# seceq/zkir

Hardware: AMD Instinct MI355X
Metric: trace rows/sec (2^20-cycle fib: execution-trace fill + BabyBear NTT/LDE + Poseidon2 Merkle commitment) (higher is better)
Workload: dtype u32 (Baby Bear, 31-bit modular) / u64 trace words

## Files before the change

### zkir_amd/build.py

```python
from __future__ import annotations

import os
import subprocess
import sys

HERE = os.path.dirname(os.path.abspath(__file__))
CSRC = os.path.join(HERE, "csrc")
OUT = os.path.join(HERE, "libzkir_amd.so")
OBJ = os.path.join(HERE, "build")

HOST_SOURCES = ["interp.cpp", "hashes.cpp", "verify.cpp"]
HIP_SOURCES = ["trace_fill.hip", "witness.hip", "ntt.hip", "stark.hip", "memcheck.hip", "abi.hip"]
HEADERS = ["host.h", "hashcall.h", "babybear.h", "poseidon2.h", "air.h", "stark_prove.inl", os.path.join("..", "..", "include", "zkir_amd.h"), os.path.join("..", "..", "include", "zkir_amd_experimental.h")]

HIPCC = os.environ.get("HIPCC", "/opt/rocm/bin/hipcc")
ARCH = "gfx950"
COMMON = ["-O3", "-std=c++17", "-fPIC", "-Wall", "-Wno-unused-function"]
EXTRA = {"stark.hip": ["-mllvm", "-amdgpu-sched-strategy=max-ilp"]}


def sources_sha16() -> str:
    import hashlib
    h = hashlib.sha256()
    for name in sorted(HIP_SOURCES + [x for x in HEADERS if not x.startswith("..")]):
# ... 22 lines not shown
        else:
            cmd = [HIPCC, "-x", "c++", *COMMON, "-march=x86-64-v2", *defines, "-c", src, "-o", obj]
        subprocess.check_call(cmd)
    out = os.path.join(HERE, "variants", f"libzkir_amd_{tag}.so")
    subprocess.check_call([HIPCC, f"--offload-arch={ARCH}", "-shared", "-fPIC", "-o", out, *objs])
    return out


PROBE_SRC = os.path.join(HERE, "..", "tests", "hip", "arith_probe.hip")
PROBE_OUT = os.path.join(HERE, "..", "tests", "hip", "libzkir_arith_probe.so")


def build_probe(force: bool = False, verbose: bool = False) -> str:
    src, out = os.path.normpath(PROBE_SRC), os.path.normpath(PROBE_OUT)
    deps = [os.path.join(CSRC, "babybear.h"), os.path.join(CSRC, "poseidon2.h")]
    if force or _newer(src, out, deps):
        cmd = [HIPCC, f"--offload-arch={ARCH}", *COMMON, *EXTRA["stark.hip"], "-shared", src, "-o", out]
        if verbose:
            print(" ".join(cmd), flush=True)
        subprocess.check_call(cmd)
    return out


def build(force: bool = False, verbose: bool = False) -> str:
    os.makedirs(OBJ, exist_ok=True)
    deps = [os.path.normpath(os.path.join(CSRC, h)) for h in HEADERS]
    objs, cmds = [], []
    for name in HOST_SOURCES + HIP_SOURCES:
        src = os.path.join(CSRC, name)
        obj = os.path.join(OBJ, name + ".o")
        objs.append(obj)
        if force or _newer(src, obj, deps):
            if name.endswith(".hip"):
                cmds.append([HIPCC, f"--offload-arch={ARCH}", *COMMON, *EXTRA.get(name, []), "-c", src, "-o", obj])
            else:
                cmds.append([HIPCC, "-x", "c++", *COMMON, "-march=x86-64-v2", "-c", src, "-o", obj])
    if cmds:
        from concurrent.futures import ThreadPoolExecutor
        def run(cmd):
            if verbose:
                print(" ".join(cmd), flush=True)
            subprocess.check_call(cmd)
        with ThreadPoolExecutor(max_workers=int(os.environ.get("ZKIR_BUILD_JOBS", "4"))) as ex:
            list(ex.map(run, cmds))
    if force or any(_newer(o, OUT, []) for o in objs):
        cmd = [HIPCC, f"--offload-arch={ARCH}", "-shared", "-fPIC", "-o", OUT, *objs]
        if verbose:
            print(" ".join(cmd), flush=True)
        subprocess.check_call(cmd)
    build_probe(force, verbose)
    return OUT


if __name__ == "__main__":
    print(build(force="--force" in sys.argv, verbose=True))
```

### zkir_amd/csrc/babybear.h

```cpp
#pragma once
#include <cstdint>

#if defined(__HIPCC__)
#define BB_HD __host__ __device__ __forceinline__
#else
#define BB_HD inline
#endif

namespace bb {

constexpr uint32_t P = 0x78000001u;
constexpr uint32_t NEG_PINV = 0x77FFFFFFu;
constexpr uint32_t R1 = 0x0FFFFFFEu;
constexpr uint32_t R2 = 0x45DDDDE3u;
constexpr uint32_t GEN = 31u;
constexpr uint32_t ROOT27 = 0x1A427A41u;
constexpr uint32_t W_EXT = 11u;

BB_HD uint32_t add(uint32_t a, uint32_t b) { const uint32_t s = a + b, d = s - P; return d < s ? d : s; }
BB_HD uint32_t sub(uint32_t a, uint32_t b) { const uint32_t d = a - b, e = d + P; return e < d ? e : d; }
BB_HD uint32_t neg(uint32_t a) { return a ? P - a : 0u; }
BB_HD uint32_t dbl(uint32_t a) { return add(a, a); }
BB_HD uint32_t mont_mul(uint32_t a, uint32_t b) {
  const uint64_t t = (uint64_t)a * b;
// ... 75 lines not shown
  return (uint32_t)((acc + (uint64_t)m * P) >> 32);
}
BB_HD int32_t smont_mul(int32_t a, int32_t b) {
  const int64_t t = (int64_t)a * b;
  const int32_t m = (int32_t)((uint32_t)t * NEG_PINV);
  return (int32_t)(((uint64_t)t + (uint64_t)((int64_t)m * (int64_t)P)) >> 32);
}
BB_HD int32_t smont_mul_add(int32_t a, int32_t b, uint64_t c) {
  const uint64_t t = (uint64_t)((int64_t)a * b) + c;
  const int32_t m = (int32_t)((uint32_t)t * NEG_PINV);
  return (int32_t)((t + (uint64_t)((int64_t)m * (int64_t)P)) >> 32);
}
BB_HD int32_t smont_reduce_wide(int64_t acc) {
  const int32_t m = (int32_t)((uint32_t)acc * NEG_PINV);
  return (int32_t)(((uint64_t)acc + (uint64_t)((int64_t)m * (int64_t)P)) >> 32);
}
BB_HD int64_t sacc_add(int64_t acc, int32_t x) {
#if defined(__HIP_DEVICE_COMPILE__)
  int64_t r;
  asm("v_mad_i64_i32 %0, vcc, %1, 1, %2" : "=v"(r) : "v"(x), "v"(acc) : "vcc");
  return r;
#else
  return acc + x;
#endif
}
BB_HD uint32_t to_mont(uint32_t a) { return mont_mul(a, R2); }
BB_HD uint32_t from_mont(uint32_t a) { return mont_mul(a, 1u); }
BB_HD uint32_t mul(uint32_t a, uint32_t b) { return mont_mul(mont_mul(a, b), R2); }
BB_HD uint32_t pow(uint32_t a, uint64_t e) {
  uint32_t r = R1, b = to_mont(a);
  while (e) { if (e & 1) r = mont_mul(r, b); b = mont_mul(b, b); e >>= 1; }
  return from_mont(r);
}
BB_HD uint32_t inv(uint32_t a) { return pow(a, P - 2); }
BB_HD uint32_t root_of_unity(int log_n) { uint32_t w = ROOT27; for (int i = log_n; i < 27; i++) w = mul(w, w); return w; }

struct E4 { uint32_t c[4]; };
BB_HD E4 e_add(const E4& a, const E4& b) { return E4{{add(a.c[0], b.c[0]), add(a.c[1], b.c[1]), add(a.c[2], b.c[2]), add(a.c[3], b.c[3])}}; }
BB_HD E4 e_sub(const E4& a, const E4& b) { return E4{{sub(a.c[0], b.c[0]), sub(a.c[1], b.c[1]), sub(a.c[2], b.c[2]), sub(a.c[3], b.c[3])}}; }
BB_HD E4 e_mul_m(const E4& a, const E4& b) {
  constexpr uint32_t W11M = (uint32_t)((11ull * R1) % P);
  const uint32_t a0 = a.c[0], a1 = a.c[1], a2 = a.c[2], a3 = a.c[3], b0 = b.c[0], b1 = b.c[1], b2 = b.c[2], b3 = b.c[3];
  const uint32_t t4 = add(add(mont_mul(a1, b3), mont_mul(a2, b2)), mont_mul(a3, b1));
  const uint32_t t5 = add(mont_mul(a2, b3), mont_mul(a3, b2));
  const uint32_t t6 = mont_mul(a3, b3);
  E4 r;
// ... 28 lines not shown
```

### zkir_amd/csrc/ntt.hip

```cpp
#include <hip/hip_runtime.h>

#include <atomic>
#include <cstdlib>
#include <mutex>
#include <type_traits>

#include "../../include/zkir_amd.h"
#include "../../include/zkir_amd_experimental.h"
#include "babybear.h"
#include "host.h"

namespace {

constexpr int NT = 256;
__device__ __forceinline__ uint32_t bitrev(uint32_t x, int bits) { return bits == 0 ? 0u : __brev(x) >> (32 - bits); }

template <int K, int N, class F>
__device__ __forceinline__ void static_for(F&& f) {
  if constexpr (K < N) { f(std::integral_constant<int, K>{}); static_for<K + 1, N>(f); }
}

using u32x4 = uint32_t __attribute__((ext_vector_type(4)));
__device__ __forceinline__ u32x4 ld4(const uint4* p) { return *reinterpret_cast<const u32x4*>(p); }
__device__ __forceinline__ void st4(uint4* p, u32x4 v) { *reinterpret_cast<u32x4*>(p) = v; }

__device__ __forceinline__ void wave_sync_lds() { asm volatile("s_waitcnt lgkmcnt(0)" ::: "memory"); }

__device__ __forceinline__ uint4 add4(uint4 a, uint4 b) { return make_uint4(bb::add(a.x, b.x), bb::add(a.y, b.y), bb::add(a.z, b.z), bb::add(a.w, b.w)); }
__device__ __forceinline__ uint4 sub4(uint4 a, uint4 b) { return make_uint4(bb::sub(a.x, b.x), bb::sub(a.y, b.y), bb::sub(a.z, b.z), bb::sub(a.w, b.w)); }
__device__ __forceinline__ uint4 addl4(uint4 a, uint4 b) { return make_uint4(a.x + b.x, a.y + b.y, a.z + b.z, a.w + b.w); }
__device__ __forceinline__ uint4 subl4(uint4 a, uint4 b) { return make_uint4(a.x - b.x + bb::P, a.y - b.y + bb::P, a.z - b.z + bb::P, a.w - b.w + bb::P); }
__device__ __forceinline__ uint4 mul4(uint4 a, uint32_t w) { return make_uint4(bb::mont_mul(a.x, w), bb::mont_mul(a.y, w), bb::mont_mul(a.z, w), bb::mont_mul(a.w, w)); }

__device__ __forceinline__ void dif4(uint4& x0, uint4& x1, uint4& x2, uint4& x3, uint32_t wA, uint32_t wB, uint32_t w2) {
  const uint4 y0 = add4(x0, x2), y2 = mul4(subl4(x0, x2), wA);
  const uint4 y1 = add4(x1, x3), y3 = mul4(subl4(x1, x3), wB);
  x0 = add4(y0, y1); x1 = mul4(subl4(y0, y1), w2);
  x2 = add4(y2, y3); x3 = mul4(subl4(y2, y3), w2);
}
__device__ __forceinline__ void dit4(uint4& x0, uint4& x1, uint4& x2, uint4& x3, uint32_t w1, uint32_t w2, uint32_t w2i) {
  const uint4 t1 = mul4(x1, w1), t3 = mul4(x3, w1);
  const uint4 y0 = add4(x0, t1), y1 = sub4(x0, t1), y2 = addl4(x2, t3), y3 = subl4(x2, t3);
  const uint4 u2 = mul4(y2, w2), u3 = mul4(y3, w2i);
  x0 = add4(y0, u2); x2 = sub4(y0, u2); x1 = add4(y1, u3); x3 = sub4(y1, u3);
}

template <bool DIT>
__global__ __launch_bounds__(NT) void ntt_stage_kernel(uint4* __restrict__ data, uint64_t blk_u4, int L, int s0, const uint32_t* __restrict__ tw) {
  uint4* x = data + (uint64_t)blockIdx.y * blk_u4;
  const uint64_t item = (uint64_t)blockIdx.x * NT + threadIdx.x;
  const uint32_t n = 1u << L;
  if (item >= (uint64_t)n) return;
  const uint32_t t = (uint32_t)(item >> 1), h = (uint32_t)(item & 1);
  uint32_t p, stride, w;
  if (DIT) { stride = 1u << s0; const uint32_t hi = t >> s0, lo = t & (stride - 1); p = (hi << (s0 + 1)) + lo; w = tw[lo << (L - s0 - 1)]; }
  else { stride = n >> (s0 + 1); const uint32_t hi = t / stride, lo = t % stride; p = hi * (n >> s0) + lo; w = tw[lo << s0]; }
  const uint4 a = x[(uint64_t)p * 2 + h], b = x[(uint64_t)(p + stride) * 2 + h];
  if (DIT) { const uint4 tt = mul4(b, w); x[(uint64_t)p * 2 + h] = add4(a, tt); x[(uint64_t)(p + stride) * 2 + h] = sub4(a, tt); }
  else { x[(uint64_t)p * 2 + h] = add4(a, b); x[(uint64_t)(p + stride) * 2 + h] = mul4(subl4(a, b), w); }
}

struct TraceSrc01 { zkir_trace_columns t; uint64_t n_real; };
__device__ __forceinline__ u32x4 trace_quad01(const TraceSrc01& q, uint32_t blk, uint32_t half, uint64_t i) {
  const bool pad = i >= q.n_real;
  const uint64_t src = pad ? q.n_real - 1 : i;
  u32x4 r;
  if (blk == 0 && half == 0) {
    const uint64_t pcv = q.t.pc[src];
    r.x = (uint32_t)((q.t.cycle[src] + (i - src)) % bb::P); r.y = (uint32_t)(pcv & 0xFFFFF); r.z = (uint32_t)((pcv >> 20) & 0xFFFFF); r.w = (uint32_t)(pcv >> 40);
  } else if (blk == 0) {
    const uint32_t w = q.t.instruction[src];
    r.x = w & 0x7F; r.y = (w >> 7) & 0xF; r.z = (w >> 11) & 0xF; r.w = (w >> 15) & 0xF;
  } else {
    auto limbs = [&](int g, uint32_t out[3]) {
      const uint64_t o = (uint64_t)g * q.t.reg_stride + src;
      const uint64_t v = q.t.registers[o];
      const int bits = q.t.reg_state[o] ? 30 : 20;
      const uint64_t mask = (1ull << bits) - 1;
      out[0] = (uint32_t)(v & mask); out[1] = (uint32_t)((v >> bits) & mask); out[2] = (uint32_t)(v >> (2 * bits));
    };
    uint32_t a[3], b[3];
    if (half == 0) { limbs(1, a); r.x = q.t.instruction[src] >> 19; r.y = a[0]; r.z = a[1]; r.w = a[2]; }
    else { limbs(2, a); limbs(3, b); r.x = a[0]; r.y = a[1]; r.z = a[2]; r.w = b[0]; }
  }
  return r;
}

template <bool DIT, int R, int C, int NTH, bool FUSED = false>
__global__ __launch_bounds__(NTH) void ntt_strided_r4_kernel(uint4* __restrict__ data, uint64_t blk_u4, uint32_t tiles_per_block, uint32_t total, int L, int s0,
                                                              const uint32_t* __restrict__ tw, const uint32_t* __restrict__ small, int log_small, uint32_t j4_m, TraceSrc01 fsrc = TraceSrc01{}) {
  constexpr int B = 2 * R;
  constexpr uint32_t POS = 1u << (B + C), QUADS = POS / 4, CMASK = (1u << C) - 1, PLANE = POS + 4;
  constexpr uint32_t MOVES = 2 * POS / NTH;
  static_assert(QUADS % NTH == 0 && NTH % (1 << C) == 0 && (2 * POS) % NTH == 0, "tile / thread geometry");
  extern __shared__ uint4 lds4[];
  const uint32_t n = 1u << L;
  const uint32_t stride_mid = DIT ? (1u << s0) : (n >> (s0 + B));
  const uint32_t lo_tiles = stride_mid >> C;
  auto geometry = [&](uint32_t w, uint4*& x, uint32_t& base, uint32_t& lo0) {
    const uint32_t tile = w % tiles_per_block;
    x = data + (uint64_t)(w / tiles_per_block) * blk_u4;
    const uint32_t hi = tile / lo_tiles;
    lo0 = (tile % lo_tiles) << C;
    base = (DIT ? (hi << (s0 + B)) : hi * (n >> s0)) + lo0;
  };
  static_assert(QUADS == NTH, "one quad per lane and round");
  u32x4 pre[MOVES];
  uint4* x; uint32_t base, lo0;
  uint32_t w = blockIdx.x;
  if (w >= total) return;
  uint32_t sm[R];
#pragma unroll
  for (int r = 0; r < R; r++) {
    const int b = 2 * r;
    const uint32_t qq = threadIdx.x >> C;
    if (!DIT) { const int lg = B - 2 - b; sm[r] = small[(qq & ((1u << lg) - 1)) << (log_small - (B - b))]; }
    else sm[r] = small[(qq & ((1u << b) - 1)) << (log_small - (b + 2))];
// ... 37 lines not shown
    }
#pragma unroll
    for (int r = 0; r < R; r++) {
      const int b = 2 * r;
#pragma unroll
      for (uint32_t k = 0; k < QUADS / NTH; k++) {
        const uint32_t q = threadIdx.x + k * NTH;
        const uint32_t lo_l = q & CMASK, qq = q >> C;
        uint32_t i0, d, wa, wb, wc;
        if (!DIT) {
          const int lg = B - 2 - b;
          const uint32_t h2 = 1u << lg, mid_lo = qq & (h2 - 1), mid_hi = qq >> lg;
          i0 = ((((mid_hi << (lg + 2)) | mid_lo)) << C) | lo_l; d = h2 << C;
          wa = bb::mont_mul(tp[r], sm[r]);
          wb = bb::mont_mul(wa, j4_m); wc = bb::mont_mul(wa, wa);
        } else {
          const uint32_t dm = 1u << b, mid_lo = qq & (dm - 1), mid_hi = qq >> b;
          i0 = ((((mid_hi << (b + 2)) | mid_lo)) << C) | lo_l; d = dm << C;
          wb = bb::mont_mul(tp[r], sm[r]);
          wa = bb::mont_mul(wb, wb); wc = bb::mont_mul(wb, j4_m);
        }
        uint4* pl0 = lds4; uint4* pl1 = lds4 + PLANE;
        uint4 x0 = pl0[i0], x1 = pl0[i0 + d], x2 = pl0[i0 + 2 * d], x3 = pl0[i0 + 3 * d];
        uint4 y0 = pl1[i0], y1 = pl1[i0 + d], y2 = pl1[i0 + 2 * d], y3 = pl1[i0 + 3 * d];
        if (!DIT) dif4(x0, x1, x2, x3, wa, wb, wc); else dit4(x0, x1, x2, x3, wa, wb, wc);
        pl0[i0] = x0; pl0[i0 + d] = x1; pl0[i0 + 2 * d] = x2; pl0[i0 + 3 * d] = x3;
        if (!DIT) dif4(y0, y1, y2, y3, wa, wb, wc); else dit4(y0, y1, y2, y3, wa, wb, wc);
        pl1[i0] = y0; pl1[i0 + d] = y1; pl1[i0 + 2 * d] = y2; pl1[i0 + 3 * d] = y3;
      }
      const bool wave_local = !DIT ? (r + 1 < R && B - 2 - b <= 6 - C) : (r + 1 < R && b + 2 <= 6 - C);
      if (wave_local) wave_sync_lds(); else __syncthreads();
    }
#pragma unroll
    for (uint32_t k = 0; k < MOVES; k++) {
      const uint32_t e = threadIdx.x + k * NTH, row = e >> (C + 1), wv = e & ((2u << C) - 1);
      x[((uint64_t)base + (uint64_t)row * stride_mid) * 2 + wv] = lds4[(wv & 1) * PLANE + ((row << C) | (wv >> 1))];
    }
    if (wn >= total) break;
    w = wn; x = xn; base = base_n; lo0 = lo0_n;
  }
}

template <bool DIT, int S>
__global__ __launch_bounds__(NT) void ntt_reg_kernel(uint4* __restrict__ data, uint64_t blk_u4, int L, int s0, const uint32_t* __restrict__ tw, uint32_t r4_m, uint32_t r8_m,
                                                       uint32_t r8_3_m) {
  constexpr int E = 1 << S;
  const uint32_t n = 1u << L;
  uint4* x = data + (uint64_t)blockIdx.y * blk_u4;
  const uint64_t item = (uint64_t)blockIdx.x * NT + threadIdx.x;
  if (item >= ((uint64_t)n >> S) * 2) return;
  const uint32_t t = (uint32_t)(item >> 1), h = (uint32_t)(item & 1);
  const uint32_t d = DIT ? (1u << s0) : (n >> (s0 + S));
  const uint32_t hi = t / d, lo = t % d;
  const uint64_t base = ((uint64_t)hi * d * E + lo) * 2 + h;
// ... 42 lines not shown
    } else {
      const uint32_t f1 = bb::mont_mul(Uf, r4_m);
#pragma unroll
      for (int g = 0; g < 4; g += 2) { const uint4 tt = mul4(v[g + 1], Um); const uint4 a = v[g]; v[g] = add4(a, tt); v[g + 1] = sub4(a, tt); }
      { const uint4 tt = mul4(v[2], Uf); const uint4 a = v[0]; v[0] = add4(a, tt); v[2] = sub4(a, tt); }
      { const uint4 tt = mul4(v[3], f1); const uint4 a = v[1]; v[1] = add4(a, tt); v[3] = sub4(a, tt); }
    }
  }
#pragma unroll
  for (int k = 0; k < E; k++) x[base + (uint64_t)k * d * 2] = v[k];
}

inline unsigned cu_count() {
  static std::mutex mu;
  static unsigned cached[64] = {};
  int dev = 0;
  if (hipGetDevice(&dev) != hipSuccess || dev < 0 || dev >= 64) return 256u;
  std::lock_guard<std::mutex> lk(mu);
  if (!cached[dev]) { hipDeviceProp_t p; cached[dev] = hipGetDeviceProperties(&p, dev) == hipSuccess && p.multiProcessorCount > 0 ? (unsigned)p.multiProcessorCount : 256u; }
  return cached[dev];
}
inline int persist() { static const int v = getenv("ZKIR_NTT_PERSIST") ? atoi(getenv("ZKIR_NTT_PERSIST")) : 1; return v; }

template <bool DIT, int R, int C, int NTH, bool FUSED = false>
void launch_strided_r4(uint32_t* data, uint64_t n, uint32_t n_blocks, int L, int s0, const uint32_t* tw, const uint32_t* small, int log_small, uint32_t j4_m, hipStream_t s,
                       const TraceSrc01* fsrc = nullptr) {
  constexpr size_t lds = 16u * 2 * ((1u << (2 * R + C)) + 4);
  auto k = ntt_strided_r4_kernel<DIT, R, C, NTH, FUSED>;
  static std::atomic<uint64_t> attr_done{0};
  int dev = 0; (void)hipGetDevice(&dev);
  const uint64_t bit = 1ull << (dev & 63);
  if (!(attr_done.load(std::memory_order_relaxed) & bit)) { (void)hipFuncSetAttribute(reinterpret_cast<const void*>(k), hipFuncAttributeMaxDynamicSharedMemorySize, (int)lds); attr_done.fetch_or(bit); }
  const uint32_t tiles = (uint32_t)(n >> (2 * R + C)), total = tiles * n_blocks;
  const unsigned per_cu = (unsigned)((160u << 10) / lds) > 0 ? (unsigned)((160u << 10) / lds) : 1u;
  unsigned grid = persist() ? cu_count() * (per_cu > 8 ? 8 : per_cu) : total;
  if (grid > total) grid = total;
  hipLaunchKernelGGL(k, dim3(grid), dim3(NTH), lds, s, (uint4*)data, 2 * n, tiles, total, L, s0, tw, small, log_small, j4_m, fsrc ? *fsrc : TraceSrc01{});
}

inline int strided_c() { static const int c = getenv("ZKIR_NTT_C") ? atoi(getenv("ZKIR_NTT_C")) : 2; return c; }

template <bool DIT>
void run_strided_stages(uint32_t* data, uint64_t n, uint32_t n_blocks, int L, int s0, int stages, const uint32_t* tw, const uint32_t* small, int log_small, uint32_t j4_m,
                        uint32_t r8_m, uint32_t r8_3_m, hipStream_t s) {
  while (stages > 0) {
    int take;
    if (stages >= 10 && stages != 11) take = 10;
    else if (stages == 11) take = 8;
    else if (stages == 9) take = 6;
    else if (stages == 7) take = 4;
    else if (stages == 5) take = 3;
    else take = stages;
    switch (take) {
      case 10:
        if (strided_c() == 2) launch_strided_r4<DIT, 5, 2, 1024>(data, n, n_blocks, L, s0, tw, small, log_small, j4_m, s);
        else launch_strided_r4<DIT, 5, 1, 512>(data, n, n_blocks, L, s0, tw, small, log_small, j4_m, s);
        break;
      case 8: launch_strided_r4<DIT, 4, 3, 512>(data, n, n_blocks, L, s0, tw, small, log_small, j4_m, s); break;
      case 6: launch_strided_r4<DIT, 3, 4, 256>(data, n, n_blocks, L, s0, tw, small, log_small, j4_m, s); break;
      case 4: launch_strided_r4<DIT, 2, 5, 128>(data, n, n_blocks, L, s0, tw, small, log_small, j4_m, s); break;
      case 3:
        hipLaunchKernelGGL((ntt_reg_kernel<DIT, 3>), dim3((unsigned)(((n >> 3) * 2 + NT - 1) / NT), n_blocks), dim3(NT), 0, s, (uint4*)data, 2 * n, L, s0, tw, j4_m, r8_m, r8_3_m);
        break;
      case 2:
        hipLaunchKernelGGL((ntt_reg_kernel<DIT, 2>), dim3((unsigned)(((n >> 2) * 2 + NT - 1) / NT), n_blocks), dim3(NT), 0, s, (uint4*)data, 2 * n, L, s0, tw, j4_m, r8_m, r8_3_m);
        break;
      default:
        hipLaunchKernelGGL(ntt_stage_kernel<DIT>, dim3((unsigned)((n + NT - 1) / NT), n_blocks), dim3(NT), 0, s, (uint4*)data, 2 * n, L, s0, tw);
        break;
    }
    s0 += take; stages -= take;
  }
}

__global__ __launch_bounds__(NT) void lde_small_kernel(const uint32_t* __restrict__ in, uint32_t* __restrict__ out, int L, const uint32_t* __restrict__ small_inv,
                                                        const uint32_t* __restrict__ small_fwd, const uint32_t* __restrict__ g_lo, const uint32_t* __restrict__ g_hi) {
  extern __shared__ uint32_t lds[];
  const uint32_t n = 1u << L;
  const uint32_t* x = in + (uint64_t)blockIdx.x * n * 8;
  uint32_t* y = out + (uint64_t)blockIdx.x * 2 * n * 8;
  for (int c = 0; c < 8; c++) {
    for (uint32_t e = threadIdx.x; e < n; e += NT) lds[e] = x[(uint64_t)e * 8 + c];
    __syncthreads();
// ... 11 lines not shown
    uint32_t v[2];
    int cnt = 0;
    for (uint32_t e = threadIdx.x; e < n; e += NT) { const uint32_t k = bitrev(e, L); v[cnt++] = bb::mont_mul(bb::mont_mul(lds[e], g_lo[k & 1023]), g_hi[k >> 10]); }
    __syncthreads();
    cnt = 0;
    for (uint32_t e = threadIdx.x; e < n; e += NT) { lds[2 * e] = v[cnt]; lds[2 * e + 1] = v[cnt]; cnt++; }
    __syncthreads();
    for (int s = 1; s <= L; s++) {
      const uint32_t half = 1u << s;
      for (uint32_t q = threadIdx.x; q < n; q += NT) {
        const uint32_t r_lo = q & (half - 1), r_hi = q >> s;
        const uint32_t ia = (r_hi << (s + 1)) | r_lo, ib = ia + half;
        const uint32_t a = lds[ia], t = bb::mont_mul(lds[ib], small_fwd[r_lo << (L - s)]);
        lds[ia] = bb::add(a, t); lds[ib] = bb::sub(a, t);
      }
      __syncthreads();
    }
    for (uint32_t e = threadIdx.x; e < 2 * n; e += NT) y[(uint64_t)e * 8 + c] = lds[e];
    __syncthreads();
  }
}

constexpr int MID_NT = 512;
__global__ __launch_bounds__(MID_NT) void lde_middle_r4_kernel(const uint4* __restrict__ in, uint4* __restrict__ out, uint32_t chunks_per_block, uint32_t total, int L,
                                                                const uint32_t* __restrict__ small_inv, const uint32_t* __restrict__ small_fwd,
                                                                const uint32_t* __restrict__ g_lo, const uint32_t* __restrict__ g_hi, uint32_t j4_inv_m, uint32_t j4_fwd_m) {
  constexpr int Bm = 10;
  constexpr uint32_t APL = 1024;
  __shared__ uint4 A[2 * APL];
  __shared__ uint4 Bf[2048];
  const uint32_t n = 1u << L, t = threadIdx.x;
  uint32_t w = blockIdx.x;
  if (w >= total) return;
  uint32_t tw_i[5], tw_f[5];
#pragma unroll
  for (int r = 0; r < 5; r++) {
    const int lg = 8 - 2 * r;
    tw_i[r] = small_inv[((t & 255) & ((1u << lg) - 1)) << (2 * r)];
    const int sft = 2 * r + 1;
    tw_f[r] = small_fwd[(t & ((1u << sft) - 1)) << (Bm - sft - 1)];
  }
  u32x4 pre[4];
  uint32_t glo[4], ghi[4];
  auto fetch = [&](uint32_t ww) {
    const uint4* x = in + ((uint64_t)(ww / chunks_per_block) * n + ((uint64_t)(ww % chunks_per_block) << Bm)) * 2;
#pragma unroll
    for (int k = 0; k < 4; k++) pre[k] = ld4(&x[t + k * MID_NT]);
// ... 21 lines not shown
        const int lg = 8 - 2 * r;
        const uint32_t h2 = 1u << lg, lo = q & (h2 - 1), hi = q >> lg;
        const uint32_t i0 = (hi << (lg + 2)) | lo;
        const uint32_t wA = tw_i[r];
        const uint32_t wB = bb::mont_mul(wA, j4_inv_m), w2 = bb::mont_mul(wA, wA);
        uint4 x0 = a[i0], x1 = a[i0 + h2], x2 = a[i0 + 2 * h2], x3 = a[i0 + 3 * h2];
        dif4(x0, x1, x2, x3, wA, wB, w2);
        if (r == 4) {
          x0 = mul4(x0, gs[0]); x1 = mul4(x1, gs[1]); x2 = mul4(x2, gs[2]); x3 = mul4(x3, gs[3]);
        }
        a[i0] = x0; a[i0 + h2] = x1; a[i0 + 2 * h2] = x2; a[i0 + 3 * h2] = x3;
        if (r >= 1 && r < 4) wave_sync_lds(); else __syncthreads();
      }
    }
#pragma unroll 1
    for (int h = 0; h < 2; h++) {
      const uint4* a = A + h * APL;
      uint4* F = h == 0 ? Bf : A;
#pragma unroll
      for (int r = 0; r < 5; r++) {
        const int s = 2 * r + 1;
        const uint32_t lo = t & ((1u << s) - 1), hi = t >> s;
        const uint32_t i0 = (hi << (s + 2)) | lo, d = 1u << s;
        const uint32_t w2 = tw_f[r];
        const uint32_t w1 = bb::mont_mul(w2, w2), w2i = bb::mont_mul(w2, j4_fwd_m);
        uint4 x0, x1, x2, x3;
        if (r == 0) {
          x0 = a[i0 >> 1]; x1 = a[(i0 + d) >> 1]; x2 = a[(i0 + 2 * d) >> 1]; x3 = a[(i0 + 3 * d) >> 1];
          __syncthreads();
        } else { x0 = F[i0]; x1 = F[i0 + d]; x2 = F[i0 + 2 * d]; x3 = F[i0 + 3 * d]; }
        dit4(x0, x1, x2, x3, w1, w2, w2i);
        F[i0] = x0; F[i0 + d] = x1; F[i0 + 2 * d] = x2; F[i0 + 3 * d] = x3;
        if (r < 2) wave_sync_lds(); else __syncthreads();
      }
    }
#pragma unroll
    for (int k = 0; k < 4; k++) { const uint32_t e = t + k * MID_NT; y[((uint64_t)2 * base + e) * 2] = Bf[e]; y[((uint64_t)2 * base + e) * 2 + 1] = A[e]; }
    __syncthreads();
    if (wn >= total) break;
    w = wn;
  }
}

}

namespace zkir {

void lde_run(const LdeTables& t, uint32_t* in, uint32_t n_blocks, uint32_t* out, void* stream) {
  hipStream_t s = (hipStream_t)stream;
  const int L = t.log_n;
  const uint32_t N = 1u << L;
  static const uint32_t j4_inv_m = bb::to_mont(bb::inv(bb::root_of_unity(2))), j4_fwd_m = bb::to_mont(bb::root_of_unity(2));
  static const uint32_t r8_fwd = bb::root_of_unity(3), r8_inv = bb::inv(r8_fwd);
  static const uint32_t r8_inv_m = bb::to_mont(r8_inv), r8_inv3_m = bb::to_mont(bb::mul(bb::mul(r8_inv, r8_inv), r8_inv));
  static const uint32_t r8_fwd_m = bb::to_mont(r8_fwd), r8_fwd3_m = bb::to_mont(bb::mul(bb::mul(r8_fwd, r8_fwd), r8_fwd));
  if (L < 10) {
    hipLaunchKernelGGL(lde_small_kernel, dim3(n_blocks), dim3(NT), (8u << L), s, in, out, L, t.small_inv, t.small_fwd, t.g_lo, t.g_hi);
    return;
  }
  run_strided_stages<false>(in, N, n_blocks, L, 0, L - 10, t.tw_inv, t.small_inv, 10, j4_inv_m, r8_inv_m, r8_inv3_m, s);
  {
    const uint32_t chunks = N >> 10, total = chunks * n_blocks;
    unsigned grid = persist() ? cu_count() * 2 : total;
    if (grid > total) grid = total;
    hipLaunchKernelGGL(lde_middle_r4_kernel, dim3(grid), dim3(MID_NT), 0, s, (const uint4*)in, (uint4*)out, chunks, total, L, t.small_inv, t.small_fwd, t.g_lo, t.g_hi,
                       j4_inv_m, j4_fwd_m);
  }
  run_strided_stages<true>(out, (uint64_t)2 * N, n_blocks, L + 1, 11, L - 10, t.tw_fwd, t.small_fwd, 11, j4_fwd_m, r8_fwd_m, r8_fwd3_m, s);
}


bool strided_variant_run(const LdeTables& t, uint32_t* data, uint32_t n_blocks, int variant, bool dit, void* stream) {
  hipStream_t s = (hipStream_t)stream;
  const int L = dit ? t.log_n + 1 : t.log_n;
  if (t.log_n < 20) return false;
  const uint64_t n = (uint64_t)1 << L;
  static const uint32_t j4_inv_m = bb::to_mont(bb::inv(bb::root_of_unity(2))), j4_fwd_m = bb::to_mont(bb::root_of_unity(2));
  const uint32_t* tw = dit ? t.tw_fwd : t.tw_inv; const uint32_t* sm = dit ? t.small_fwd : t.small_inv;
  const int ls = dit ? 11 : 10; const uint32_t j4 = dit ? j4_fwd_m : j4_inv_m; const int s0 = dit ? 11 : 0;
#define ZKIR_VARIANT(R, C, NTH) do { if (dit) launch_strided_r4<true, R, C, NTH>(data, n, n_blocks, L, s0, tw, sm, ls, j4, s); else launch_strided_r4<false, R, C, NTH>(data, n, n_blocks, L, s0, tw, sm, ls, j4, s); } while (0)
  switch (variant) {
    case 0: ZKIR_VARIANT(5, 2, 1024); break;
    case 1: ZKIR_VARIANT(5, 1, 512); break;
    case 2: ZKIR_VARIANT(4, 3, 512); break;
    case 3: ZKIR_VARIANT(4, 2, 256); break;
    case 4: ZKIR_VARIANT(3, 4, 256); break;
    default: return false;
  }
#undef ZKIR_VARIANT
  return true;
}

bool lde_run_fused01(const LdeTables& t, const zkir_trace_columns* trace, uint64_t n_real, uint32_t* in, uint32_t n_blocks, uint32_t* out, void* stream) {
  hipStream_t s = (hipStream_t)stream;
  const int L = t.log_n;
  if (L < 20 || L == 21 || n_blocks < 3 || strided_c() != 2) return false;
  const uint32_t N = 1u << L;
  static const uint32_t j4_inv_m = bb::to_mont(bb::inv(bb::root_of_unity(2))), j4_fwd_m = bb::to_mont(bb::root_of_unity(2));
  static const uint32_t r8_fwd = bb::root_of_unity(3), r8_inv = bb::inv(r8_fwd);
  static const uint32_t r8_inv_m = bb::to_mont(r8_inv), r8_inv3_m = bb::to_mont(bb::mul(bb::mul(r8_inv, r8_inv), r8_inv));
  static const uint32_t r8_fwd_m = bb::to_mont(r8_fwd), r8_fwd3_m = bb::to_mont(bb::mul(bb::mul(r8_fwd, r8_fwd), r8_fwd));
  const TraceSrc01 src{*trace, n_real};
  launch_strided_r4<false, 5, 2, 1024, true>(in, N, 2, L, 0, t.tw_inv, t.small_inv, 10, j4_inv_m, s, &src);
  launch_strided_r4<false, 5, 2, 1024>(in + (uint64_t)2 * N * 8, N, n_blocks - 2, L, 0, t.tw_inv, t.small_inv, 10, j4_inv_m, s);
  if (L - 10 > 10) run_strided_stages<false>(in, N, n_blocks, L, 10, L - 20, t.tw_inv, t.small_inv, 10, j4_inv_m, r8_inv_m, r8_inv3_m, s);
  {
    const uint32_t chunks = N >> 10, total = chunks * n_blocks;
    unsigned grid = persist() ? cu_count() * 2 : total;
    if (grid > total) grid = total;
    hipLaunchKernelGGL(lde_middle_r4_kernel, dim3(grid), dim3(MID_NT), 0, s, (const uint4*)in, (uint4*)out, chunks, total, L, t.small_inv, t.small_fwd, t.g_lo, t.g_hi,
                       j4_inv_m, j4_fwd_m);
  }
  run_strided_stages<true>(out, (uint64_t)2 * N, n_blocks, L + 1, 11, L - 10, t.tw_fwd, t.small_fwd, 11, j4_fwd_m, r8_fwd_m, r8_fwd3_m, s);
  return true;
}

}
```

Before: 185.6 million.

## Use signed wide-accumulator radix-4 DIT butterflies with deferred canonicalisation in forward NTT

Replaces the forward (DIT) radix-4 butterfly in the strided and LDE-middle kernels with a signed 64-bit accumulation scheme. Twiddles are centred to signed values and products are accumulated with v_mad_i64_i32, and reductions happen only twice per butterfly instead of after every add/sub. Outputs stay in a signed redundant range and are canonicalised only on the final round of the last forward pass. Results go to LDS through hand-written ds_write2 stores. The aim is fewer modular add/sub/reduce instructions, at the cost of complex bound reasoning, more inline asm, and sched barriers that may limit compiler scheduling. It also adds an NTT probe build target.

```diff
diff --git a/zkir_amd/build.py b/zkir_amd/build.py
--- a/zkir_amd/build.py
+++ b/zkir_amd/build.py
@@ -68,6 +68,20 @@
     return out
 
 
+NTT_PROBE_SRC = os.path.join(HERE, "..", "tests", "hip", "ntt_probe.hip")
+NTT_PROBE_OUT = os.path.join(HERE, "..", "tests", "hip", "libzkir_ntt_probe.so")
+
+
+def build_ntt_probe(force: bool = False, verbose: bool = False) -> str:
+    src, out = os.path.normpath(NTT_PROBE_SRC), os.path.normpath(NTT_PROBE_OUT)
+    if force or _newer(src, out, [os.path.join(CSRC, "babybear.h")]):
+        cmd = [HIPCC, f"--offload-arch={ARCH}", *COMMON, *EXTRA.get("ntt.hip", []), "-shared", src, "-o", out]
+        if verbose:
+            print(" ".join(cmd), flush=True)
+        subprocess.check_call(cmd)
+    return out
+
+
 def build(force: bool = False, verbose: bool = False) -> str:
     os.makedirs(OBJ, exist_ok=True)
     deps = [os.path.normpath(os.path.join(CSRC, h)) for h in HEADERS]
@@ -95,6 +109,7 @@
             print(" ".join(cmd), flush=True)
         subprocess.check_call(cmd)
     build_probe(force, verbose)
+    build_ntt_probe(force, verbose)
     return OUT
 
 
diff --git a/zkir_amd/csrc/babybear.h b/zkir_amd/csrc/babybear.h
--- a/zkir_amd/csrc/babybear.h
+++ b/zkir_amd/csrc/babybear.h
@@ -121,6 +121,76 @@
   return r;
 #else
   return acc + x;
+#endif
+}
+namespace wq {
+constexpr int64_t W_MAX = (P - 1) / 2;
+constexpr int64_t X_ANY = (int64_t)1 << 31;
+constexpr int64_t RED_DOMAIN = (int64_t)(((uint64_t)1 << 63) - ((uint64_t)P << 31));
+constexpr int64_t red_bound(int64_t acc) { return (acc + ((int64_t)P << 31)) >> 32; }
+constexpr int64_t layer1_acc_bound(int64_t x) { return x * ((int64_t)R1 + W_MAX); }
+constexpr int64_t final_acc_bound(int64_t x) { return layer1_acc_bound(x) + red_bound(layer1_acc_bound(x)) * W_MAX; }
+constexpr int64_t out_bound(int64_t x) { return red_bound(final_acc_bound(x)); }
+constexpr int64_t OUT_ANY = out_bound(X_ANY);
+constexpr int64_t OUT_CHAINED = out_bound(OUT_ANY);
+static_assert(layer1_acc_bound(X_ANY) < RED_DOMAIN && final_acc_bound(X_ANY) < RED_DOMAIN, "wide quad: an accumulator leaves the reduction's domain");
+static_assert(OUT_ANY < X_ANY, "wide quad: outputs must fit int32 (closed under iteration)");
+static_assert(OUT_CHAINED < (int64_t)P, "wide quad: a chained round's outputs must lie in (-p, p) for scanon_pp");
+static_assert(out_bound(OUT_CHAINED) <= OUT_CHAINED, "wide quad: the chained bound must not grow");
+}
+BB_HD int32_t scentre(uint32_t w) { return (int32_t)(w > (uint32_t)wq::W_MAX ? w - P : w); }
+BB_HD uint32_t scanon(int32_t x) {
+  int32_t y = x + ((x >> 31) & (int32_t)P);
+  y += (y >> 31) & (int32_t)P;
+  return reduce_2p((uint32_t)y);
+}
+BB_HD uint32_t scanon_pp(uint32_t x) { const uint32_t e = x + P; return e < x ? e : x; }
+struct WideTw { int32_t w1, nw1, w2, nw2, w2i, nw2i; };
+BB_HD WideTw wide_twiddles(uint32_t w1, uint32_t w2, uint32_t w2i) {
+  const int32_t a = scentre(w1), b = scentre(w2), c = scentre(w2i);
+  return WideTw{a, -a, b, -b, c, -c};
+}
+BB_HD void dit4_wide_col(uint32_t& x0, uint32_t& x1, uint32_t& x2, uint32_t& x3, const WideTw& t, int64_t* acc = nullptr) {
+  const int64_t p0 = (int64_t)(int32_t)x0 * (int32_t)R1, p2 = (int64_t)(int32_t)x2 * (int32_t)R1;
+  const int64_t y0 = p0 + (int64_t)(int32_t)x1 * t.w1, y1 = p0 + (int64_t)(int32_t)x1 * t.nw1;
+  const int64_t y2 = p2 + (int64_t)(int32_t)x3 * t.w1, y3 = p2 + (int64_t)(int32_t)x3 * t.nw1;
+  const int32_t r2 = smont_reduce_wide(y2), r3 = smont_reduce_wide(y3);
+  const int64_t z0 = y0 + (int64_t)r2 * t.w2, z2 = y0 + (int64_t)r2 * t.nw2, z1 = y1 + (int64_t)r3 * t.w2i, z3 = y1 + (int64_t)r3 * t.nw2i;
+  if (acc) { acc[0] = y0; acc[1] = y1; acc[2] = y2; acc[3] = y3; acc[4] = z0; acc[5] = z1; acc[6] = z2; acc[7] = z3; }
+  x0 = (uint32_t)smont_reduce_wide(z0); x1 = (uint32_t)smont_reduce_wide(z1); x2 = (uint32_t)smont_reduce_wide(z2); x3 = (uint32_t)smont_reduce_wide(z3);
+}
+BB_HD void dit4_wide_x2(uint32_t& a0, uint32_t& a1, uint32_t& a2, uint32_t& a3, uint32_t& b0, uint32_t& b1, uint32_t& b2, uint32_t& b3, const WideTw& t) {
+#if defined(__HIP_DEVICE_COMPILE__)
+  int64_t ya0, ya1, ya2, ya3, yb0, yb1, yb2, yb3;
+  asm("v_mad_i64_i32 %0, vcc, %8, %18, 0\n\tv_mad_i64_i32 %2, vcc, %10, %18, 0\n\tv_mad_i64_i32 %4, vcc, %12, %18, 0\n\tv_mad_i64_i32 %6, vcc, %14, %18, 0\n\t"
+      "v_mad_i64_i32 %1, vcc, %9, %17, %0\n\tv_mad_i64_i32 %3, vcc, %11, %17, %2\n\tv_mad_i64_i32 %5, vcc, %13, %17, %4\n\tv_mad_i64_i32 %7, vcc, %15, %17, %6\n\t"
+      "v_mad_i64_i32 %0, vcc, %9, %16, %0\n\tv_mad_i64_i32 %2, vcc, %11, %16, %2\n\tv_mad_i64_i32 %4, vcc, %13, %16, %4\n\tv_mad_i64_i32 %6, vcc, %15, %16, %6"
+      : "=&v"(ya0), "=&v"(ya1), "=&v"(ya2), "=&v"(ya3), "=&v"(yb0), "=&v"(yb1), "=&v"(yb2), "=&v"(yb3)
+      : "v"(a0), "v"(a1), "v"(a2), "v"(a3), "v"(b0), "v"(b1), "v"(b2), "v"(b3), "v"(t.w1), "v"(t.nw1), "s"(R1) : "vcc");
+  {
+    const uint32_t m0 = (uint32_t)ya2 * NEG_PINV, m1 = (uint32_t)ya3 * NEG_PINV, m2 = (uint32_t)yb2 * NEG_PINV, m3 = (uint32_t)yb3 * NEG_PINV;
+    asm("v_mad_i64_i32 %0, vcc, %4, %8, %0\n\tv_mad_i64_i32 %1, vcc, %5, %8, %1\n\tv_mad_i64_i32 %2, vcc, %6, %8, %2\n\tv_mad_i64_i32 %3, vcc, %7, %8, %3"
+        : "+v"(ya2), "+v"(ya3), "+v"(yb2), "+v"(yb3) : "v"(m0), "v"(m1), "v"(m2), "v"(m3), "s"(P) : "vcc");
+  }
+  const int32_t ra2 = (int32_t)(ya2 >> 32), ra3 = (int32_t)(ya3 >> 32), rb2 = (int32_t)(yb2 >> 32), rb3 = (int32_t)(yb3 >> 32);
+  int64_t za2, za3, zb2, zb3;
+  asm("v_mad_i64_i32 %4, vcc, %8, %13, %0\n\tv_mad_i64_i32 %5, vcc, %9, %15, %1\n\tv_mad_i64_i32 %6, vcc, %10, %13, %2\n\tv_mad_i64_i32 %7, vcc, %11, %15, %3\n\t"
+      "v_mad_i64_i32 %0, vcc, %8, %12, %0\n\tv_mad_i64_i32 %1, vcc, %9, %14, %1\n\tv_mad_i64_i32 %2, vcc, %10, %12, %2\n\tv_mad_i64_i32 %3, vcc, %11, %14, %3"
+      : "+v"(ya0), "+v"(ya1), "+v"(yb0), "+v"(yb1), "=&v"(za2), "=&v"(za3), "=&v"(zb2), "=&v"(zb3)
+      : "v"(ra2), "v"(ra3), "v"(rb2), "v"(rb3), "v"(t.w2), "v"(t.nw2), "v"(t.w2i), "v"(t.nw2i) : "vcc");
+  {
+    const uint32_t m0 = (uint32_t)ya0 * NEG_PINV, m1 = (uint32_t)ya1 * NEG_PINV, m2 = (uint32_t)za2 * NEG_PINV, m3 = (uint32_t)za3 * NEG_PINV;
+    const uint32_t m4 = (uint32_t)yb0 * NEG_PINV, m5 = (uint32_t)yb1 * NEG_PINV, m6 = (uint32_t)zb2 * NEG_PINV, m7 = (uint32_t)zb3 * NEG_PINV;
+    asm("v_mad_i64_i32 %0, vcc, %8, %16, %0\n\tv_mad_i64_i32 %1, vcc, %9, %16, %1\n\tv_mad_i64_i32 %2, vcc, %10, %16, %2\n\tv_mad_i64_i32 %3, vcc, %11, %16, %3\n\t"
+        "v_mad_i64_i32 %4, vcc, %12, %16, %4\n\tv_mad_i64_i32 %5, vcc, %13, %16, %5\n\tv_mad_i64_i32 %6, vcc, %14, %16, %6\n\tv_mad_i64_i32 %7, vcc, %15, %16, %7"
+        : "+v"(ya0), "+v"(ya1), "+v"(za2), "+v"(za3), "+v"(yb0), "+v"(yb1), "+v"(zb2), "+v"(zb3)
+        : "v"(m0), "v"(m1), "v"(m2), "v"(m3), "v"(m4), "v"(m5), "v"(m6), "v"(m7), "s"(P) : "vcc");
+  }
+  a0 = (uint32_t)(ya0 >> 32); a1 = (uint32_t)(ya1 >> 32); a2 = (uint32_t)(za2 >> 32); a3 = (uint32_t)(za3 >> 32);
+  b0 = (uint32_t)(yb0 >> 32); b1 = (uint32_t)(yb1 >> 32); b2 = (uint32_t)(zb2 >> 32); b3 = (uint32_t)(zb3 >> 32);
+#else
+  dit4_wide_col(a0, a1, a2, a3, t);
+  dit4_wide_col(b0, b1, b2, b3, t);
 #endif
 }
 BB_HD uint32_t to_mont(uint32_t a) { return mont_mul(a, R2); }
diff --git a/zkir_amd/csrc/ntt.hip b/zkir_amd/csrc/ntt.hip
--- a/zkir_amd/csrc/ntt.hip
+++ b/zkir_amd/csrc/ntt.hip
@@ -43,6 +43,33 @@
   const uint4 y0 = add4(x0, t1), y1 = sub4(x0, t1), y2 = addl4(x2, t3), y3 = subl4(x2, t3);
   const uint4 u2 = mul4(y2, w2), u3 = mul4(y3, w2i);
   x0 = add4(y0, u2); x2 = sub4(y0, u2); x1 = add4(y1, u3); x3 = sub4(y1, u3);
+}
+
+__device__ __forceinline__ uint32_t lds_addr(const void* p) {
+  uint32_t a = (uint32_t)(uintptr_t)(__attribute__((address_space(3))) const void*)p;
+  asm volatile("" : "+v"(a));
+  return a;
+}
+template <int OFF>
+__device__ __forceinline__ void lds_st2x4(uint32_t p0, uint32_t p1, uint32_t p2, uint32_t p3, uint32_t a0, uint32_t b0, uint32_t a1, uint32_t b1, uint32_t a2, uint32_t b2, uint32_t a3, uint32_t b3) {
+  asm volatile("ds_write2_b32 %0, %4, %5 offset0:%12 offset1:%13\n\tds_write2_b32 %1, %6, %7 offset0:%12 offset1:%13\n\t"
+               "ds_write2_b32 %2, %8, %9 offset0:%12 offset1:%13\n\tds_write2_b32 %3, %10, %11 offset0:%12 offset1:%13"
+               :: "v"(p0), "v"(p1), "v"(p2), "v"(p3), "v"(a0), "v"(b0), "v"(a1), "v"(b1), "v"(a2), "v"(b2), "v"(a3), "v"(b3),
+                  "n"(OFF), "n"(OFF + 1) : "memory");
+}
+template <int OFF>
+__device__ __forceinline__ void dit4w_pair(uint32_t p0, uint32_t p1, uint32_t p2, uint32_t p3, const uint4& x0, const uint4& x1, const uint4& x2, const uint4& x3, const bb::WideTw& t, bool canon) {
+  uint32_t a0, a1, a2, a3, b0, b1, b2, b3;
+  if constexpr (OFF == 0) { a0 = x0.x; a1 = x1.x; a2 = x2.x; a3 = x3.x; b0 = x0.y; b1 = x1.y; b2 = x2.y; b3 = x3.y; }
+  else { a0 = x0.z; a1 = x1.z; a2 = x2.z; a3 = x3.z; b0 = x0.w; b1 = x1.w; b2 = x2.w; b3 = x3.w; }
+  bb::dit4_wide_x2(a0, a1, a2, a3, b0, b1, b2, b3, t);
+  if (canon) { a0 = bb::scanon_pp(a0); a1 = bb::scanon_pp(a1); a2 = bb::scanon_pp(a2); a3 = bb::scanon_pp(a3); b0 = bb::scanon_pp(b0); b1 = bb::scanon_pp(b1); b2 = bb::scanon_pp(b2); b3 = bb::scanon_pp(b3); }
+  lds_st2x4<OFF>(p0, p1, p2, p3, a0, b0, a1, b1, a2, b2, a3, b3);
+  __builtin_amdgcn_sched_barrier(0);
+}
+__device__ __forceinline__ void dit4w_store(uint32_t p0, uint32_t p1, uint32_t p2, uint32_t p3, const uint4& x0, const uint4& x1, const uint4& x2, const uint4& x3, const bb::WideTw& t, bool canon) {
+  dit4w_pair<0>(p0, p1, p2, p3, x0, x1, x2, x3, t, canon);
+  dit4w_pair<2>(p0, p1, p2, p3, x0, x1, x2, x3, t, canon);
 }
 
 template <bool DIT>
@@ -86,13 +113,14 @@
   return r;
 }
 
-template <bool DIT, int R, int C, int NTH, bool FUSED = false>
+template <bool DIT, int R, int C, int NTH, bool FUSED = false, bool CANON = false>
 __global__ __launch_bounds__(NTH) void ntt_strided_r4_kernel(uint4* __restrict__ data, uint64_t blk_u4, uint32_t tiles_per_block, uint32_t total, int L, int s0,
                                                               const uint32_t* __restrict__ tw, const uint32_t* __restrict__ small, int log_small, uint32_t j4_m, TraceSrc01 fsrc = TraceSrc01{}) {
   constexpr int B = 2 * R;
   constexpr uint32_t POS = 1u << (B + C), QUADS = POS / 4, CMASK = (1u << C) - 1, PLANE = POS + 4;
   constexpr uint32_t MOVES = 2 * POS / NTH;
   static_assert(QUADS % NTH == 0 && NTH % (1 << C) == 0 && (2 * POS) % NTH == 0, "tile / thread geometry");
+  static_assert(!CANON || (DIT && R >= 2), "only a forward pass canonicalises, and its last round must be a chained one (bb::wq::OUT_CHAINED < p)");
   extern __shared__ uint4 lds4[];
   const uint32_t n = 1u << L;
   const uint32_t stride_mid = DIT ? (1u << s0) : (n >> (s0 + B));
@@ -176,14 +204,26 @@
         }
         uint4* pl0 = lds4; uint4* pl1 = lds4 + PLANE;
         uint4 x0 = pl0[i0], x1 = pl0[i0 + d], x2 = pl0[i0 + 2 * d], x3 = pl0[i0 + 3 * d];
-        uint4 y0 = pl1[i0], y1 = pl1[i0 + d], y2 = pl1[i0 + 2 * d], y3 = pl1[i0 + 3 * d];
-        if (!DIT) dif4(x0, x1, x2, x3, wa, wb, wc); else dit4(x0, x1, x2, x3, wa, wb, wc);
-        pl0[i0] = x0; pl0[i0 + d] = x1; pl0[i0 + 2 * d] = x2; pl0[i0 + 3 * d] = x3;
-        if (!DIT) dif4(y0, y1, y2, y3, wa, wb, wc); else dit4(y0, y1, y2, y3, wa, wb, wc);
-        pl1[i0] = y0; pl1[i0 + d] = y1; pl1[i0 + 2 * d] = y2; pl1[i0 + 3 * d] = y3;
+        if constexpr (!DIT) {
+          uint4 y0 = pl1[i0], y1 = pl1[i0 + d], y2 = pl1[i0 + 2 * d], y3 = pl1[i0 + 3 * d];
+          dif4(x0, x1, x2, x3, wa, wb, wc);
+          pl0[i0] = x0; pl0[i0 + d] = x1; pl0[i0 + 2 * d] = x2; pl0[i0 + 3 * d] = x3;
+          dif4(y0, y1, y2, y3, wa, wb, wc);
+          pl1[i0] = y0; pl1[i0 + d] = y1; pl1[i0 + 2 * d] = y2; pl1[i0 + 3 * d] = y3;
+        } else {
+          const bb::WideTw wt = bb::wide_twiddles(wa, wb, wc);
+          const bool canon = CANON && r == R - 1;
+          const uint32_t ad = lds_addr(&pl0[i0]), dB = d * 16, pB = PLANE * 16;
+          dit4w_pair<0>(ad, ad + dB, ad + 2 * dB, ad + 3 * dB, x0, x1, x2, x3, wt, canon);
+          dit4w_pair<2>(ad, ad + dB, ad + 2 * dB, ad + 3 * dB, x0, x1, x2, x3, wt, canon);
+          const uint4 y0 = pl1[i0], y1 = pl1[i0 + d], y2 = pl1[i0 + 2 * d], y3 = pl1[i0 + 3 * d];
+          dit4w_store(ad + pB, ad + pB + dB, ad + pB + 2 * dB, ad + pB + 3 * dB, y0, y1, y2, y3, wt, canon);
+        }
       }
       const bool wave_local = !DIT ? (r + 1 < R && B - 2 - b <= 6 - C) : (r + 1 < R && b + 2 <= 6 - C);
-      if (wave_local) wave_sync_lds(); else __syncthreads();
+      if (DIT) wave_sync_lds();
+      if (!wave_local) __syncthreads();
+      else if (!DIT) wave_sync_lds();
     }
 #pragma unroll
     for (uint32_t k = 0; k < MOVES; k++) {
@@ -272,11 +312,11 @@
 }
 inline int persist() { static const int v = getenv("ZKIR_NTT_PERSIST") ? atoi(getenv("ZKIR_NTT_PERSIST")) : 1; return v; }
 
-template <bool DIT, int R, int C, int NTH, bool FUSED = false>
+template <bool DIT, int R, int C, int NTH, bool FUSED = false, bool CANON = false>
 void launch_strided_r4(uint32_t* data, uint64_t n, uint32_t n_blocks, int L, int s0, const uint32_t* tw, const uint32_t* small, int log_small, uint32_t j4_m, hipStream_t s,
                        const TraceSrc01* fsrc = nullptr) {
   constexpr size_t lds = 16u * 2 * ((1u << (2 * R + C)) + 4);
-  auto k = ntt_strided_r4_kernel<DIT, R, C, NTH, FUSED>;
+  auto k = ntt_strided_r4_kernel<DIT, R, C, NTH, FUSED, CANON>;
   static std::atomic<uint64_t> attr_done{0};
   int dev = 0; (void)hipGetDevice(&dev);
   const uint64_t bit = 1ull << (dev & 63);
@@ -287,6 +327,15 @@
   if (grid > total) grid = total;
   hipLaunchKernelGGL(k, dim3(grid), dim3(NTH), lds, s, (uint4*)data, 2 * n, tiles, total, L, s0, tw, small, log_small, j4_m, fsrc ? *fsrc : TraceSrc01{});
 }
+
+template <bool DIT, int R, int C, int NTH>
+void launch_strided_r4_fwd(bool canon, uint32_t* data, uint64_t n, uint32_t n_blocks, int L, int s0, const uint32_t* tw, const uint32_t* small, int log_small, uint32_t j4_m, hipStream_t s) {
+  if constexpr (DIT) {
+    if (canon) { launch_strided_r4<true, R, C, NTH, false, true>(data, n, n_blocks, L, s0, tw, small, log_small, j4_m, s); return; }
+  }
+  launch_strided_r4<DIT, R, C, NTH>(data, n, n_blocks, L, s0, tw, small, log_small, j4_m, s);
+}
+constexpr bool first_pass_is_r4(int stages) { return stages >= 4 && stages != 5; }
 
 inline int strided_c() { static const int c = getenv("ZKIR_NTT_C") ? atoi(getenv("ZKIR_NTT_C")) : 2; return c; }
 
@@ -301,14 +350,15 @@
     else if (stages == 7) take = 4;
     else if (stages == 5) take = 3;
     else take = stages;
+    const bool canon = DIT && !first_pass_is_r4(stages - take);
     switch (take) {
       case 10:
-        if (strided_c() == 2) launch_strided_r4<DIT, 5, 2, 1024>(data, n, n_blocks, L, s0, tw, small, log_small, j4_m, s);
-        else launch_strided_r4<DIT, 5, 1, 512>(data, n, n_blocks, L, s0, tw, small, log_small, j4_m, s);
+        if (strided_c() == 2) launch_strided_r4_fwd<DIT, 5, 2, 1024>(canon, data, n, n_blocks, L, s0, tw, small, log_small, j4_m, s);
+        else launch_strided_r4_fwd<DIT, 5, 1, 512>(canon, data, n, n_blocks, L, s0, tw, small, log_small, j4_m, s);
         break;
-      case 8: launch_strided_r4<DIT, 4, 3, 512>(data, n, n_blocks, L, s0, tw, small, log_small, j4_m, s); break;
-      case 6: launch_strided_r4<DIT, 3, 4, 256>(data, n, n_blocks, L, s0, tw, small, log_small, j4_m, s); break;
-      case 4: launch_strided_r4<DIT, 2, 5, 128>(data, n, n_blocks, L, s0, tw, small, log_small, j4_m, s); break;
+      case 8: launch_strided_r4_fwd<DIT, 4, 3, 512>(canon, data, n, n_blocks, L, s0, tw, small, log_small, j4_m, s); break;
+      case 6: launch_strided_r4_fwd<DIT, 3, 4, 256>(canon, data, n, n_blocks, L, s0, tw, small, log_small, j4_m, s); break;
+      case 4: launch_strided_r4_fwd<DIT, 2, 5, 128>(canon, data, n, n_blocks, L, s0, tw, small, log_small, j4_m, s); break;
       case 3:
         hipLaunchKernelGGL((ntt_reg_kernel<DIT, 3>), dim3((unsigned)(((n >> 3) * 2 + NT - 1) / NT), n_blocks), dim3(NT), 0, s, (uint4*)data, 2 * n, L, s0, tw, j4_m, r8_m, r8_3_m);
         break;
@@ -366,7 +416,8 @@
 }
 
 constexpr int MID_NT = 512;
-__global__ __launch_bounds__(MID_NT) void lde_middle_r4_kernel(const uint4* __restrict__ in, uint4* __restrict__ out, uint32_t chunks_per_block, uint32_t total, int L,
+template <bool CANON>
+__global__ __launch_bounds__(MID_NT, 4) void lde_middle_r4_kernel(const uint4* __restrict__ in, uint4* __restrict__ out, uint32_t chunks_per_block, uint32_t total, int L,
                                                                 const uint32_t* __restrict__ small_inv, const uint32_t* __restrict__ small_fwd,
                                                                 const uint32_t* __restrict__ g_lo, const uint32_t* __restrict__ g_hi, uint32_t j4_inv_m, uint32_t j4_fwd_m) {
   constexpr int Bm = 10;
@@ -434,16 +485,18 @@
         const int s = 2 * r + 1;
         const uint32_t lo = t & ((1u << s) - 1), hi = t >> s;
         const uint32_t i0 = (hi << (s + 2)) | lo, d = 1u << s;
-        const uint32_t w2 = tw_f[r];
+        uint32_t w2 = tw_f[r];
+        asm volatile("" : "+v"(w2));
         const uint32_t w1 = bb::mont_mul(w2, w2), w2i = bb::mont_mul(w2, j4_fwd_m);
         uint4 x0, x1, x2, x3;
         if (r == 0) {
           x0 = a[i0 >> 1]; x1 = a[(i0 + d) >> 1]; x2 = a[(i0 + 2 * d) >> 1]; x3 = a[(i0 + 3 * d) >> 1];
           __syncthreads();
         } else { x0 = F[i0]; x1 = F[i0 + d]; x2 = F[i0 + 2 * d]; x3 = F[i0 + 3 * d]; }
-        dit4(x0, x1, x2, x3, w1, w2, w2i);
-        F[i0] = x0; F[i0 + d] = x1; F[i0 + 2 * d] = x2; F[i0 + 3 * d] = x3;
-        if (r < 2) wave_sync_lds(); else __syncthreads();
+        const uint32_t ad = lds_addr(&F[i0]), dB = d * 16;
+        dit4w_store(ad, ad + dB, ad + 2 * dB, ad + 3 * dB, x0, x1, x2, x3, bb::wide_twiddles(w1, w2, w2i), CANON && r == 4);
+        wave_sync_lds();
+        if (r >= 2) __syncthreads();
       }
     }
 #pragma unroll
@@ -452,6 +505,15 @@
     if (wn >= total) break;
     w = wn;
   }
+}
+
+void launch_middle(const zkir::LdeTables& t, const uint32_t* in, uint32_t n_blocks, uint32_t* out, uint32_t j4_inv_m, uint32_t j4_fwd_m, hipStream_t s) {
+  const int L = t.log_n;
+  const uint32_t chunks = (1u << L) >> 10, total = chunks * n_blocks;
+  unsigned grid = persist() ? cu_count() * 2 : total;
+  if (grid > total) grid = total;
+  auto k = first_pass_is_r4(L - 10) ? lde_middle_r4_kernel<false> : lde_middle_r4_kernel<true>;
+  hipLaunchKernelGGL(k, dim3(grid), dim3(MID_NT), 0, s, (const uint4*)in, (uint4*)out, chunks, total, L, t.small_inv, t.small_fwd, t.g_lo, t.g_hi, j4_inv_m, j4_fwd_m);
 }
 
 }
@@ -472,11 +534,7 @@
   }
   run_strided_stages<false>(in, N, n_blocks, L, 0, L - 10, t.tw_inv, t.small_inv, 10, j4_inv_m, r8_inv_m, r8_inv3_m, s);
   {
-    const uint32_t chunks = N >> 10, total = chunks * n_blocks;
-    unsigned grid = persist() ? cu_count() * 2 : total;
-    if (grid > total) grid = total;
-    hipLaunchKernelGGL(lde_middle_r4_kernel, dim3(grid), dim3(MID_NT), 0, s, (const uint4*)in, (uint4*)out, chunks, total, L, t.small_inv, t.small_fwd, t.g_lo, t.g_hi,
-                       j4_inv_m, j4_fwd_m);
+    launch_middle(t, in, n_blocks, out, j4_inv_m, j4_fwd_m, s);
   }
   run_strided_stages<true>(out, (uint64_t)2 * N, n_blocks, L + 1, 11, L - 10, t.tw_fwd, t.small_fwd, 11, j4_fwd_m, r8_fwd_m, r8_fwd3_m, s);
 }
@@ -517,11 +575,7 @@
   launch_strided_r4<false, 5, 2, 1024>(in + (uint64_t)2 * N * 8, N, n_blocks - 2, L, 0, t.tw_inv, t.small_inv, 10, j4_inv_m, s);
   if (L - 10 > 10) run_strided_stages<false>(in, N, n_blocks, L, 10, L - 20, t.tw_inv, t.small_inv, 10, j4_inv_m, r8_inv_m, r8_inv3_m, s);
   {
-    const uint32_t chunks = N >> 10, total = chunks * n_blocks;
-    unsigned grid = persist() ? cu_count() * 2 : total;
-    if (grid > total) grid = total;
-    hipLaunchKernelGGL(lde_middle_r4_kernel, dim3(grid), dim3(MID_NT), 0, s, (const uint4*)in, (uint4*)out, chunks, total, L, t.small_inv, t.small_fwd, t.g_lo, t.g_hi,
-                       j4_inv_m, j4_fwd_m);
+    launch_middle(t, in, n_blocks, out, j4_inv_m, j4_fwd_m, s);
   }
   run_strided_stages<true>(out, (uint64_t)2 * N, n_blocks, L + 1, 11, L - 10, t.tw_fwd, t.small_fwd, 11, j4_fwd_m, r8_fwd_m, r8_fwd3_m, s);
   return true;
```

New measurement: 180.7 million. 2.6% lower.
